# thomaspingel/neilpy

Hardware: AMD Instinct MI355X
Metric: Mcells/s through SMRF progressive_filter, 16384x16384 fp32 DEM (higher is better)
Workload: dtype f32

## Files before the change

### neilpy_amd/csrc/morph_incero.h

```cpp
#pragma once
#include "morph_ring.h"

namespace smrf {

#include "ero_inc.inc"
constexpr bool dil_cross_radii_are_rim_free() {
  for (int r = SMRF_INCERO_MIN_RADIUS; r <= SMRF_INCERO_MAX_RADIUS; ++r)
    if (smrf_dil_cross_has(4, r) != (kEroInc[r].n == 0)) return false;
  return true;
}
static_assert(dil_cross_radii_are_rim_free(), "smrf_dil_cross_has (pf_route.h) against ero_inc.inc");

enum { kIncEroPlain = 0, kIncEroMirrorSplit = 1, kIncEroMirrorCopy = 2 };
inline constexpr unsigned char kIncEroPlanKind[65] = {
    1, 1, 1, 1, 1, 1, 1, 1, 1, 1, 1, 1, 1, 1, 1, 1, 1,
    1, 1, 1, 1, 1, 1, 1, 1, 1, 1, 1, 1, 1, 1, 1, 1, 1,
    1, 1, 1, 1, 1, 1, 1, 1, 1, 1, 2, 2, 1, 1, 1, 1, 1,
    1, 1, 1, 1, 1, 1, 1, 1, 1, 1, 1, 1, 1, 1};
inline constexpr unsigned char kIncEroCrossLate[65] = {
    0, 0, 0, 0, 0, 0, 0, 0, 0, 0, 0, 0, 0, 0, 0, 0, 0,
    0, 0, 0, 0, 0, 0, 0, 0, 0, 0, 0, 0, 0, 0, 0, 0, 0,
    0, 0, 0, 0, 0, 1, 0, 0, 0, 0, 1, 1, 0, 0, 0, 1, 1,
    0, 0, 0, 0, 0, 0, 0, 0, 0, 0, 0, 0, 0, 0};
#ifndef SMRF_INCERO_MIRROR_GROUP
#define SMRF_INCERO_MIRROR_GROUP 2
#endif
constexpr int inc_ero_plan_kind(int radius) {
#ifdef SMRF_INCERO_PLAN
  return SMRF_INCERO_PLAN;
#else
  return kIncEroPlanKind[radius];
#endif
}
constexpr bool inc_ero_cross_late(int radius) {
#ifdef SMRF_INCERO_LATE
  return SMRF_INCERO_LATE;
#else
  return kIncEroCrossLate[radius] != 0;
#endif
}

template <typename T>
struct IncEroArgs {
  const T* e_prev;
  const T* last;
  T* out;
  int rows, cols;
  long long ld;
  int seg;
  int nt;
  int plain_tiles;
};

template <int R>
struct IncEroCfg {
  static constexpr int N = kEroInc[R].n;
  static constexpr int DY = kEroInc[R].reach;
  static constexpr int TW = 256, NP = 4, ROWS = 2 * NP;
  static constexpr int W = TW + 2 * DY;
  static constexpr int NPOS = (W + TW - 1) / TW;
  static constexpr int NACC = 2 * DY + ROWS;
  static constexpr int KIND = N > 0 ? inc_ero_plan_kind(R) : kIncEroPlain;
  static constexpr int NM = N / 2;
  static constexpr int G = KIND == kIncEroPlain ? 4 : SMRF_INCERO_MIRROR_GROUP;
  static constexpr int NJ = NP * N;
  static constexpr int dy(int k) { return kEroInc[R].p[k].dy; }
  static constexpr int dx(int k) { return kEroInc[R].p[k].dx; }
  static constexpr int slot(int j) { return 2 * (j / N) - dy(j % N) + DY; }
  static constexpr int mirror(int j) { return (j / N) * N + N - 1 - j % N; }
  static constexpr bool mirrored() {
    for (int k = 0; k < N; ++k)
      if (dy(k) != -dy(N - 1 - k) || dx(k) != dx(N - 1 - k) || dy(k) == 0) return false;
    return N % 2 == 0;
  }
  static constexpr short NONE = 32767;
  struct Item { short j; bool both; };
  struct Plan { short n, splits, copies; Item item[NJ > 0 ? NJ : 1]; short first[NACC]; };
  static constexpr Plan make_plan() {
    Plan pl{};
    for (int s = 0; s < NACC; ++s) pl.first[s] = NONE;
    auto emit = [&](int j, bool both) {
      for (int h = 0; h < (both ? 2 : 1); ++h)
        for (int b = 0; b < 2; ++b) {
          short& f = pl.first[slot(h ? mirror(j) : j) + b];
          if (f == NONE) f = pl.n;
        }
      pl.item[pl.n++] = Item{(short)j, both};
    };
    if constexpr (KIND == kIncEroPlain) {
      for (int s = 0; s < NACC; ++s)
        for (int j = 0; j < NJ; ++j)
          if (slot(j) == s) emit(j, false);
    } else {
      constexpr int NGR = NP * NM;
      auto jlo = [](int g) { return (g / NM) * N + NM + g % NM; };
      auto lo = [&](int g) { return slot(jlo(g)); };
      auto hi = [&](int g) { return slot(mirror(jlo(g))); };
      bool touched[NACC] = {}, done[NACC] = {};
      unsigned char state[NGR > 0 ? NGR : 1] = {};
      for (int g = 0; g < NGR; ++g) touched[lo(g)] = touched[lo(g) + 1] = touched[hi(g)] = touched[hi(g) + 1] = true;
      auto unready = [&](int g, int part) {
        int u = 0;
        for (int h = 0; h < 2; ++h)
          if (part >> h & 1)
            for (int b = 0; b < 2; ++b) {
// ... 16 lines not shown
          if (!part || unready(g, part)) continue;
          const int key = part & 1 ? lo(g) : hi(g);
          if (bg < 0 || key < bkey) bg = g, bpart = part, bkey = key;
        }
        if (bg < 0 && KIND == kIncEroMirrorSplit) {
          int bcnt = -1;
          for (int g = 0; g < NGR; ++g)
            for (int part = 1; part <= 2 && !state[g]; ++part) {
              if (unready(g, part)) continue;
              const int s = part == 1 ? lo(g) : hi(g);
              const bool was[2] = {done[s], done[s + 1]};
              done[s] = done[s + 1] = true;
              state[g] |= (unsigned char)part;
              int cnt = 0;
              for (int h = 0; h < NGR; ++h) {
                const int rest = 3 & ~state[h];
                const int a = lo(h) - s - ROWS, c = hi(h) - s - ROWS;
                if (rest && ((a >= -1 && a <= 1) || (c >= -1 && c <= 1)) && !unready(h, rest)) ++cnt;
              }
              state[g] = 0;
              done[s] = was[0], done[s + 1] = was[1];
              if (cnt > bcnt || (cnt == bcnt && s < bkey)) bg = g, bpart = part, bkey = s, bcnt = cnt;
            }
          ++pl.splits;
        } else if (bg < 0) {
          int bu = 0;
          for (int g = 0; g < NGR; ++g) {
            if (state[g]) continue;
            const int u = unready(g, 3);
            if (bg < 0 || u < bu || (u == bu && lo(g) < bkey)) bg = g, bpart = 3, bkey = lo(g), bu = u;
          }
        }
        run(bg, bpart);
        left -= bpart == 3 ? 2 : 1;
      }
    }
    return pl;
  }
  static constexpr Plan plan = make_plan();
  static constexpr int NI = plan.n;
  static constexpr int NG = (NI + G - 1) / G;
  static constexpr int gsize(int g) { const int n = NI - g * G; return n < 0 ? 0 : n > G ? G : n; }
  static constexpr bool plan_ok() {
    if (N > 0 && !mirrored()) return false;
    int seen[NJ > 0 ? NJ : 1] = {};
    for (int i = 0; i < NI; ++i) {
      ++seen[plan.item[i].j];
      if (plan.item[i].both) ++seen[mirror(plan.item[i].j)];
    }
    for (int j = 0; j < NJ; ++j)
      if (seen[j] != 1) return false;
    if (KIND == kIncEroPlain ? NI != NJ || plan.splits || plan.copies : NI != NP * NM + plan.splits) return false;
    if ((KIND == kIncEroMirrorSplit && plan.copies) || (KIND == kIncEroMirrorCopy && plan.splits)) return false;
    int late = 0;
    for (int s = 0; s < NACC; ++s) {
      int earliest = NONE, touches = 0;
      for (int i = NI - 1; i >= 0; --i)
        for (int h = 0; h < (plan.item[i].both ? 2 : 1); ++h)
          for (int b = 0; b < 2; ++b)
            if (slot(h ? mirror(plan.item[i].j) : plan.item[i].j) + b == s) { ++touches; earliest = i; }
      if (plan.first[s] != earliest) return false;
      if (touches && s + ROWS < NACC && plan.first[s + ROWS] != NONE && plan.first[s] >= plan.first[s + ROWS]) ++late;
    }
    return late == plan.copies;
  }
  static constexpr bool LATE = N > 0 && inc_ero_cross_late(R);
  static constexpr int DELTA = (ROWS - (2 * DY) % ROWS) % ROWS;
  static constexpr int LDS_CELLS = N > 0 ? 2 * NP * W : 1;
};

template <typename T, int R>
__global__ __launch_bounds__(256) void inc_erode_kernel(const IncEroArgs<T> a) {
  using C = IncEroCfg<R>;
  using T2 = typename Vec2<T>::type;
  constexpr int N = C::N, DY = C::DY, TW = C::TW, NP = C::NP, ROWS = C::ROWS, W = C::W, NPOS = C::NPOS, NACC = C::NACC, G = C::G;
  __shared__ T2 L[C::LDS_CELLS];
  const int tid = threadIdx.x;
  int bx, by;
  smrf_xcd_tile(a.plain_tiles, [] { return true; }, bx, by);
  const int x0 = bx * TW, x = x0 + tid;
  const int ys = by * a.seg, ye = min(a.rows, ys + a.seg);
  if (ys >= ye) return;
  const int xc = x < a.cols ? x : a.cols - 1;
  const int xl = smrf_fold(xc - 1, a.cols), xr = smrf_fold(xc + 1, a.cols);
  int cpos[NPOS];
  bool act[NPOS];
#pragma unroll
  for (int i = 0; i < NPOS; ++i) {
    act[i] = tid + i * TW < W;
    cpos[i] = smrf_fold(x0 - DY + tid + (act[i] ? i * TW : 0), a.cols);
  }
  T acc[NACC];
#pragma unroll
  for (int i = 0; i < NACC; ++i) acc[i] = ident<T>(false);

  static_assert(C::plan_ok(), "the batch plan");
  int o0 = ys - 2 * DY - C::DELTA;
  const int nb = (ye - o0 + ROWS - 1) / ROWS;
  RowFold rf(o0 + DY, a.rows);
  T2 pf[NP][NPOS];
  auto prefetch = [&]() {
#pragma unroll
    for (int p = 0; p < NP; ++p) {
      const T* ra = a.last + (long long)rf.at(2 * p) * a.ld;
      const T* rb = a.last + (long long)rf.at(2 * p + 1) * a.ld;
#pragma unroll
      for (int i = 0; i < NPOS; ++i)
        { pf[p][i].x = ra[cpos[i]]; pf[p][i].y = rb[cpos[i]]; }
    }
    rf.advance(ROWS);
  };
  if constexpr (N > 0) prefetch();

  T outv[ROWS];
  auto store_rows = [&](int ob) {
#pragma unroll
    for (int j = 0; j < ROWS; ++j)
      if (ob + j < ye && x < a.cols) smrf_store_out(a.out + (long long)(ob + j) * a.ld + x, outv[j], a.nt);
  };
  for (int b = 0; b < nb; ++b, o0 += ROWS) {
    const unsigned lds_b = (unsigned)(size_t)(__attribute__((address_space(3))) void*)(L + (b & 1) * NP * W + tid);
    if constexpr (N > 0) {
#pragma unroll
      for (int p = 0; p < NP; ++p)
#pragma unroll
        for (int i = 0; i < NPOS; ++i)
          lds_write2(lds_b + (unsigned)((p * W + (i < NPOS - 1 || act[i] ? i * TW : 0)) * (int)sizeof(T2)), pf[p][i]);
      lds_wait<0>();
      __syncthreads();
    }
    if (o0 - ROWS >= ys) store_rows(o0 - ROWS);
    const bool store = o0 >= ys;
    T ec[ROWS + 2], el[ROWS], er[ROWS];
    auto cross_loads = [&]() {
      RowFold rfe(o0 - 1, a.rows);
#pragma unroll
      for (int j = 0; j < ROWS + 2; ++j) {
        const T* row = a.e_prev + (long long)rfe.at(j) * a.ld;
        ec[j] = row[xc];
        if (j >= 1 && j <= ROWS) { el[j - 1] = row[xl]; er[j - 1] = row[xr]; }
      }
    };
    if constexpr (!C::LATE)
      if (store) cross_loads();
    if constexpr (N > 0) {
      __builtin_amdgcn_sched_barrier(0);
      prefetch();
      __builtin_amdgcn_sched_barrier(0);
      T old[NACC];
#pragma unroll
      for (int s = 0; s < NACC; ++s) old[s] = acc[s];
      [&]<int... S>(std::integer_sequence<int, S...>) {
        (([&] {
           if constexpr (C::plan.first[S] == C::NONE) acc[S] = S + ROWS < NACC ? old[S + ROWS] : ident<T>(false);
         }()),
         ...);
      }(std::make_integer_sequence<int, NACC>{});
      T2 rd[2 * G][2];
      auto issue = [&]<int I>(std::integral_constant<int, I>) {
        constexpr int J = C::plan.item[I].j, p = J / N, k = J % N;
        constexpr int offl = (p * W + DY - C::dx(k)) * (int)sizeof(T2), offr = (p * W + DY + C::dx(k)) * (int)sizeof(T2);
        rd[I % (2 * G)][0] = lds_read2<offl>(lds_b, T());
        rd[I % (2 * G)][1] = lds_read2<offr>(lds_b, T());
      };
      auto update = [&]<int S, int I>(std::integral_constant<int, S>, std::integral_constant<int, I>, const T& l, const T& r) {
        static_assert(S >= 0 && S < NACC, "slot outside the ring");
        if constexpr (C::plan.first[S] != I) op3_acc<false>(acc[S], l, r);
        else if constexpr (S + ROWS < NACC) acc[S] = op3<false>(old[S + ROWS], l, r);
        else acc[S] = op2<false>(l, r);
      };
      auto apply = [&]<int I>(std::integral_constant<int, I> i) {
        constexpr int s = C::slot(C::plan.item[I].j), m = C::slot(C::mirror(C::plan.item[I].j));
        update(std::integral_constant<int, s>{}, i, rd[I % (2 * G)][0].x, rd[I % (2 * G)][1].x);
        if constexpr (C::plan.item[I].both) update(std::integral_constant<int, m>{}, i, rd[I % (2 * G)][0].x, rd[I % (2 * G)][1].x);
        update(std::integral_constant<int, s + 1>{}, i, rd[I % (2 * G)][0].y, rd[I % (2 * G)][1].y);
        if constexpr (C::plan.item[I].both) update(std::integral_constant<int, m + 1>{}, i, rd[I % (2 * G)][0].y, rd[I % (2 * G)][1].y);
      };
      auto issue_group = [&]<int Gi>(std::integral_constant<int, Gi>) {
        [&]<int... I>(std::integer_sequence<int, I...>) {
          (issue(std::integral_constant<int, Gi * G + I>{}), ...);
        }(std::make_integer_sequence<int, C::gsize(Gi)>{});
      };
      auto apply_group = [&]<int Gi>(std::integral_constant<int, Gi>) {
        [&]<int... I>(std::integer_sequence<int, I...>) {
          (apply(std::integral_constant<int, Gi * G + I>{}), ...);
        }(std::make_integer_sequence<int, C::gsize(Gi)>{});
      };
      issue_group(std::integral_constant<int, 0>{});
      [&]<int... Gi>(std::integer_sequence<int, Gi...>) {
        (([&] {
           if constexpr (Gi + 1 < C::NG) {
             issue_group(std::integral_constant<int, Gi + 1>{});
             lds_wait<2 * C::gsize(Gi + 1)>();
           } else {
             lds_wait<0>();
           }
           apply_group(std::integral_constant<int, Gi>{});
         }()),
         ...);
      }(std::make_integer_sequence<int, C::NG>{});
    }
    if (store) {
      if constexpr (C::LATE) cross_loads();
#pragma unroll
      for (int j = 0; j < ROWS; ++j) {
        T m = op3<false>(ec[j + 1], el[j], er[j]);
        m = op3<false>(m, ec[j], ec[j + 2]);
        if constexpr (N > 0) m = op2<false>(m, acc[j]);
        outv[j] = m;
      }
    }
  }
  if (o0 - ROWS >= ys) store_rows(o0 - ROWS);
}

template <typename T, int R>
int inc_erode_launch(const IncEroArgs<T>& a_in, hipStream_t stream) {
  using C = IncEroCfg<R>;
  constexpr auto kern = inc_erode_kernel<T, R>;
  int resident;
  bool first;
  if (int rc = smrf_resident<kern>(C::TW, 0, resident, first)) return rc;
  if (first && smrf_sw().ring_debug)
    fprintf(stderr, "smrf inc erode: R=%d pairs=%d reach=%d LDS=%zu, %d workgroups/CU resident\n", R, C::N, C::DY,
            C::LDS_CELLS * 2 * sizeof(T), resident);
  IncEroArgs<T> a = a_in;
  const int strips = (a.cols + C::TW - 1) / C::TW;
  a.seg = smrf_seg_len(a.rows, strips, resident, smrf_sw().ring_rounds, 2 * C::DY + C::DELTA, C::ROWS, std::max(32, 4 * C::DY),
                       smrf_sw().seg_rule, a.seg);
  a.plain_tiles = smrf_sw().xcd_remap ? 0 : 1;
  dim3 grid(strips, (a.rows + a.seg - 1) / a.seg);
  hipLaunchKernelGGL(kern, grid, dim3(C::TW), 0, stream, a);
  SMRF_LAUNCH_CHECK();
  return SMRF_OK;
}

}
```

### neilpy_amd/csrc/morph_ring.h

```cpp
#pragma once
#include <algorithm>
#include <utility>

#include "smrf_common.h"

#ifndef SMRF_RING_G
#define SMRF_RING_G(ringregs) ((ringregs) > 132 ? 3 : (ringregs) > 100 ? 2 : 4)
#define SMRF_RING_G_OF(T, R, ringregs) (ring_tuned_g<T>(R) > 0 ? ring_tuned_g<T>(R) : SMRF_RING_G(ringregs))
#else
#define SMRF_RING_G_OF(T, R, ringregs) SMRF_RING_G(ringregs)
#endif
#ifndef SMRF_RING_TOP3
#define SMRF_RING_TOP3(T, R) ring_tuned_top3<T>(R)
#endif
#ifndef SMRF_RING_NP_MAX
#define SMRF_RING_NP_MAX 2
#endif
#ifndef SMRF_RING_XCD_REMAP
#define SMRF_RING_XCD_REMAP 1
#endif
#ifndef SMRF_RING_SLOPE_DEFAULT
#define SMRF_RING_SLOPE_DEFAULT 60
#endif
#ifndef SMRF_RING_OCC_DROP
// ... 313 lines not shown
  static constexpr int OCC_REG = INPLACE && SMRF_RING_INPLACE_OCC(T, R) > 0 ? SMRF_RING_INPLACE_OCC(T, R)
                                                                          : ring_occ_drop(OCC_EST, SMRF_RING_OCC_DROP_OF(T, R));
  static constexpr int WAVES = TW / 64;
  static constexpr int WG_LDS = (int)(160 * 1024 / LDS_BYTES) < 1 ? 1 : (int)(160 * 1024 / LDS_BYTES);
  static constexpr int OCC_LDS = WG_LDS * WAVES / 4 < 1 ? 1 : WG_LDS * WAVES / 4;
  static constexpr int OCC = OCC_REG < OCC_LDS ? OCC_REG : OCC_LDS;
  static constexpr int kA(int s) { int d = R - s - 2; return S::kidx(d < 0 ? -d : d); }
  static constexpr int kB(int s) { int d = R - s - 1; return S::kidx(d < 0 ? -d : d); }
  static constexpr int slot_group(int s) {
    if (s > R - 2) return NG;
    const int k = kA(s);
    return k == 0 ? 0 : (k - 1) / G;
  }
};

template <typename T, int R, int TW>
constexpr int ring_np() {
  using C1 = RingCfg<T, R, TW, 1>;
  constexpr int mx = C1::INPLACE && SMRF_RING_INPLACE_NP(T, R) > 0 ? SMRF_RING_INPLACE_NP(T, R)
                     : sizeof(T) == 4 ? SMRF_RING_NP_MAX_OF(T, R) : (ring_tuned_np_max<T>(R) / 2 < 1 ? 1 : ring_tuned_np_max<T>(R) / 2);
  constexpr int want = C1::OCC_REG * 4 / C1::WAVES < 1 ? 1 : C1::OCC_REG * 4 / C1::WAVES;
  if constexpr (mx >= 4) if (RingCfg<T, R, TW, 4>::WG_LDS >= want) return 4;
  if constexpr (mx >= 3) if (RingCfg<T, R, TW, 3>::WG_LDS >= want) return 3;
  if constexpr (mx >= 2) if (RingCfg<T, R, TW, 2>::WG_LDS >= want) return 2;
  return 1;
}
#define SMRF_RING_NP(T, R) ring_np<T, R, kRingTW>()


#ifndef SMRF_RING_BUF
#define SMRF_RING_BUF(T, R) ring_tuned_buf<T>(R)
#endif
#ifndef SMRF_RING_INPLACE_NOBUF
#define SMRF_RING_INPLACE_NOBUF(T, R) ((R) > 45)
#endif
template <typename T, int R, int TW, int NP>
constexpr bool ring_buf_on() { return SMRF_RING_BUF(T, R) && !(RingCfg<T, R, TW, NP>::INPLACE && SMRF_RING_INPLACE_NOBUF(T, R)); }
template <bool ON>
__device__ __forceinline__ int smrf_rare(int v) {
  if constexpr (ON) asm volatile("" : "+v"(v));
  return v;
}
using smrf_rsrc_t = __amdgpu_buffer_rsrc_t;
__device__ __forceinline__ smrf_rsrc_t smrf_make_rsrc(const void* p) {
  return __builtin_amdgcn_make_buffer_rsrc(const_cast<void*>(p), 0, -1, 0x00020000);
}
__device__ __forceinline__ float smrf_buf_load(smrf_rsrc_t r, unsigned voff, unsigned soff, float) {
  return __builtin_bit_cast(float, __builtin_amdgcn_raw_buffer_load_b32(r, (int)voff, (int)soff, 0));
}
__device__ __forceinline__ double smrf_buf_load(smrf_rsrc_t r, unsigned voff, unsigned soff, double) {
  return __builtin_bit_cast(double, __builtin_amdgcn_raw_buffer_load_b64(r, (int)voff, (int)soff, 0));
}
template <bool NT>
__device__ __forceinline__ void smrf_buf_store(smrf_rsrc_t r, unsigned voff, unsigned soff, float v) {
  __builtin_amdgcn_raw_buffer_store_b32(__builtin_bit_cast(unsigned, v), r, (int)voff, (int)soff, NT ? 2 : 0);
}
template <bool NT>
__device__ __forceinline__ void smrf_buf_store(smrf_rsrc_t r, unsigned voff, unsigned soff, double v) {
  typedef unsigned u2 __attribute__((ext_vector_type(2)));
  __builtin_amdgcn_raw_buffer_store_b64(__builtin_bit_cast(u2, v), r, (int)voff, (int)soff, NT ? 2 : 0);
}
__device__ __forceinline__ void smrf_buf_store_u8(smrf_rsrc_t r, unsigned voff, unsigned soff, uint8_t v) {
  __builtin_amdgcn_raw_buffer_store_b8(v, r, (int)voff, (int)soff, 0);
}

template <typename T>
__device__ __forceinline__ void smrf_store_out(T* p, T v, int nt) {
  if (nt) __builtin_nontemporal_store(v, p);
  else *p = v;
}
template <typename T>
__device__ __forceinline__ void smrf_flag_cell(const DiskArgs<T>& a, long long off, T lastval, T val) {
  const T diff = lastval - val;
  bool hit;
  if constexpr (sizeof(T) == 4) hit = diff > a.thr_lo;
  else hit = (double)diff > a.thr;
  if (a.dense) {
    a.mask[off] = hit ? 1 : 0;
    if (a.when != nullptr) a.when[off] = hit ? (uint8_t)a.widx : (uint8_t)0;
  } else if (hit) {
    a.mask[off] = 1;
    if (a.when != nullptr) a.when[off] = (uint8_t)a.widx;
  }
}

struct RowFold {
  int n, p;
  __device__ __forceinline__ RowFold(int y, int n_) : n(n_) {
    p = y % (2 * n);
    if (p < 0) p += 2 * n;
  }
  __device__ __forceinline__ int at(int i) const {
    int q = p + i;
    while (q >= 2 * n) q -= 2 * n;
    return q < n ? q : 2 * n - 1 - q;
  }
  __device__ __forceinline__ void advance(int d) {
    p += d;
    while (p >= 2 * n) p -= 2 * n;
  }
};

template <typename T, int R, bool DIL, int TW, int NP, int NPB, int OFF>
__device__ __forceinline__ void ring_base(typename Vec2<T>::type* const L, const int par, const int tid, const bool has_last,
                                          typename Vec2<T>::type (&v)[NP][RingCfg<T, R, TW, NP>::NPOS]) {
  using C = RingCfg<T, R, TW, NP>;
  using T2 = typename Vec2<T>::type;
  constexpr int WP = C::WP, NLEV = C::NLEV;
  constexpr int JB = C::JB, SB = C::slot_of(JB);
  constexpr int NA = (1 << JB) - 1;
  const unsigned lds_l = (unsigned)(size_t)(__attribute__((address_space(3))) void*)(L + tid + OFF);
  constexpr int PB = C::BASE_PB < NP ? C::BASE_PB : NP;
#pragma unroll
  for (int i = 0; i < NPB; ++i) {
    if (i < NPB - 1 || has_last) {
     const int pos = tid + OFF + i * TW;
#pragma unroll
     for (int p0 = 0; p0 < NP; p0 += PB) {
      T2 na[NP][NA];
#pragma unroll
      for (int p = p0; p < p0 + PB && p < NP; ++p) {
        const unsigned ad = lds_l + ((p * NLEV + par) * WP + i * TW) * (unsigned)sizeof(T2);
        [&]<int... Kk>(std::integer_sequence<int, Kk...>) {
          ((na[p][Kk] = lds_read2<(Kk + 1) * (int)sizeof(T2)>(ad, T())), ...);
        }(std::make_integer_sequence<int, NA>{});
      }
      lds_wait<0>();
#pragma unroll
      for (int p = p0; p < p0 + PB && p < NP; ++p) {
        const T2* n = na[p];
        T2 m = v[p][i];
        if constexpr (C::INC) {
          m.x = op2<DIL>(m.x, n[0].x); m.y = op2<DIL>(m.y, n[0].y);
          if constexpr (JB >= 2) {
            if constexpr (C::stored(1)) { constexpr int s1 = C::slot_of(1); L[(p * NLEV + s1) * WP + pos] = m; }
            m.x = op3<DIL>(m.x, n[1].x, n[2].x); m.y = op3<DIL>(m.y, n[1].y, n[2].y);
          }
          if constexpr (JB == 3) {
            if constexpr (C::stored(2)) { constexpr int s2 = C::slot_of(2); L[(p * NLEV + s2) * WP + pos] = m; }
            m.x = op3<DIL>(m.x, n[3].x, n[4].x); m.y = op3<DIL>(m.y, n[3].y, n[4].y);
            m.x = op3<DIL>(m.x, n[5].x, n[6].x); m.y = op3<DIL>(m.y, n[5].y, n[6].y);
          }
        } else {
        if constexpr (JB == 1) { m.x = op2<DIL>(m.x, n[0].x); m.y = op2<DIL>(m.y, n[0].y); }
        if constexpr (JB >= 2) {
          m.x = op3<DIL>(m.x, n[0].x, n[1].x); m.y = op3<DIL>(m.y, n[0].y, n[1].y);
          m.x = op2<DIL>(m.x, n[2].x); m.y = op2<DIL>(m.y, n[2].y);
        }
        if constexpr (JB == 3) {
          m.x = op3<DIL>(m.x, n[3].x, n[4].x); m.y = op3<DIL>(m.y, n[3].y, n[4].y);
          m.x = op3<DIL>(m.x, n[5].x, n[6].x); m.y = op3<DIL>(m.y, n[5].y, n[6].y);
        }
        }
        v[p][i] = m;
        L[(p * NLEV + SB) * WP + pos] = m;
      }
      __builtin_amdgcn_sched_barrier(0);
     }
    }
  }
}

template <typename T, int R, bool DIL, int TW, int NP, int NPB, int OFF>
__device__ __forceinline__ void ring_upper(typename Vec2<T>::type* const L, const int tid, const bool has_last,
                                           typename Vec2<T>::type (&v)[NP][RingCfg<T, R, TW, NP>::NPOS]) {
  using C = RingCfg<T, R, TW, NP>;
// ... 382 lines not shown
           constexpr int ka = C::kA(Sl), kb = C::kB(Sl);
           if constexpr ((ka - 1) / G == GI) {
             constexpr int src = Sl + 2 <= R - 2 ? Sl + 2 : R - 1 + ((Sl + 2 - (R - 1)) + 2 * P) % M;
             acc[Sl] = op3<DIL>(acc[src], ra[ka], rb[kb]);
           }
         }()), ...);
      }(std::make_integer_sequence<int, R - 1>{});
      [&]<int... Jr>(std::integer_sequence<int, Jr...>) {
        (([&] {
           constexpr int j = R - 2 - Jr;
           constexpr int ka = S::kidx(j + 1), kb = S::kidx(j);
           if constexpr ((kb - 1) / G == GI) {
             constexpr int reg = R - 1 + (j + 2 + 2 * P) % M;
             op3_acc<DIL>(acc[reg], ra[ka], rb[kb]);
           }
         }()), ...);
      }(std::make_integer_sequence<int, R - 1>{});
    };
    [&]<int... GI>(std::integer_sequence<int, GI...>) {
      (([&] { if constexpr (GI < NG) lk.template issue<GI>(); }()), ...);
    }(std::make_integer_sequence<int, D - 1>{});
    ra[0] = own[P].x;
    rb[0] = own[P].y;
    outv[2 * P] = op2<DIL>(acc[0], ra[0]);
    constexpr bool SD = C::SLOT_DELAY && NG >= 2;
    [&]<int... GI>(std::integer_sequence<int, GI...>) {
      (([&] {
         if constexpr (GI + D - 1 < NG) lk.template issue<GI + D - 1>();
         lds_wait<C::inflight_after(GI), (C::FUSE_MODE != 0)>();
         lk.template reduce<GI>();
         constexpr int GS = SD ? GI - 1 : GI;
         if constexpr (GS == (KR1 - 1) / G) outv[2 * P + 1] = op3<DIL>(acc[1], ra[KR1], rb[0]);
         if constexpr (!SD && GI == NG - 1) __builtin_amdgcn_s_setprio(0);
         if constexpr (GS >= 0) slots(std::integral_constant<int, GS>{});
       }()), ...);
    }(std::make_integer_sequence<int, NG>{});
    if constexpr (SD) {
      __builtin_amdgcn_s_setprio(0);
      if constexpr (NG - 1 == (KR1 - 1) / G) outv[2 * P + 1] = op3<DIL>(acc[1], ra[KR1], rb[0]);
      slots(std::integral_constant<int, NG - 1>{});
    }
    acc[R - 1 + (2 * P) % M] = op2<DIL>(ra[0], rb[KR1]);
    acc[R - 1 + (1 + 2 * P) % M] = rb[0];
    __builtin_amdgcn_sched_barrier(0);
  };
  [&]<int... P>(std::integer_sequence<int, P...>) {
    (pair_body(std::integral_constant<int, P>{}), ...);
  }(std::make_integer_sequence<int, NP>{});
  {
    constexpr int ROT = (2 * NP) % M;
    if constexpr (ROT != 0) {
      SMRF_MARK("turn");
      T t[M];
#pragma unroll
      for (int i = 0; i < M; ++i) t[i] = acc[R - 1 + (i + ROT) % M];
      if constexpr (sizeof(T) == 4 && SMRF_RING_TURN_ASM(T, R)) {
#pragma unroll
        for (int i = 0; i < M; ++i) asm volatile("v_mov_b32 %0, %1" : "=v"(acc[R - 1 + i]) : "v"(t[i]));
      } else {
#pragma unroll
        for (int i = 0; i < M; ++i) acc[R - 1 + i] = t[i];
      }
    }
  }
}

template <typename T, int R, bool DIL, int TW, int NP, int NPB, int OFF, typename Sync>
__device__ __forceinline__ void ring_build_consume(typename Vec2<T>::type* const L, const int par, const int tid,
                                                   const bool has_last,
                                                   typename Vec2<T>::type (&v)[NP][RingCfg<T, R, TW, NP>::NPOS],
                                                   T (&acc)[2 * R], T (&outv)[2 * NP], Sync&& phase_sync) {
  __builtin_amdgcn_s_setprio(kRingBuildPrio);
  ring_base<T, R, DIL, TW, NP, NPB, OFF>(L, par, tid, has_last, v);
  phase_sync();
  if constexpr (RingCfg<T, R, TW, NP>::J > RingCfg<T, R, TW, NP>::JB) {
    ring_upper<T, R, DIL, TW, NP, NPB, OFF>(L, tid, has_last, v);
    phase_sync();
  }
  __builtin_amdgcn_s_setprio(0);
  ring_consume<T, R, DIL, TW, NP>(L, par, tid, acc, outv);
}

#ifndef SMRF_CROSS_NP
#define SMRF_CROSS_NP(R) ((R) == 16 ? 2 : 0)
#endif
#ifndef SMRF_CROSS_OCC
#define SMRF_CROSS_OCC(R) ((R) == 36 ? 2 : 3)
#endif
template <int R, int TW, int NP>
constexpr int ring_cross_occ() {
  using C = RingCfg<float, R, TW, NP>;
  constexpr int o = SMRF_CROSS_OCC(R) > 0 ? SMRF_CROSS_OCC(R) : C::OCC_REG;
  return o < C::OCC_LDS ? o : C::OCC_LDS;
}

template <typename T, int R, bool DIL, int TW, int NP>
__global__ __launch_bounds__(TW, (RingCfg<T, R, TW, NP>::OCC))
void ring_kernel(const DiskArgs<T> a) {
  constexpr bool CROSS = false;
#include "ring_kernel_body.inc"
}

template <int R, int TW, int NP>
__global__ __launch_bounds__(TW, (ring_cross_occ<R, TW, NP>()))
void ring_cross_kernel(const DiskArgs<float> a) {
  using T = float;
  constexpr bool DIL = true, CROSS = true;
#include "ring_kernel_body.inc"
}

template <typename T, int R, bool DIL, int NP, bool CROSS = false>
int ring_launch_np(const DiskArgs<T>& a_in, hipStream_t stream, bool probe_only, int* seg_if_launched) {
  constexpr int TW = kRingTW;
  using C = RingCfg<T, R, TW, NP>;
  constexpr auto kern = [] {
    if constexpr (CROSS) return ring_cross_kernel<R, TW, NP>;
    else return ring_kernel<T, R, DIL, TW, NP>;
  }();
  constexpr int occ = [] {
    if constexpr (CROSS) return ring_cross_occ<R, TW, NP>();
    else return (int)C::OCC;
  }();
  int resident;
  bool first;
  if (int rc = smrf_resident<kern>(TW, C::LDS_BYTES, resident, first)) return rc;
  if (first && smrf_sw().ring_debug)
    fprintf(stderr, "smrf ring: R=%d %s%s NP=%d G=%d%s LDS=%zu built for %d waves/SIMD, %d workgroups/CU resident\n", R,
            sizeof(T) == 4 ? "f32" : "f64", CROSS ? " dilate of the cross" : DIL ? " dilate" : " erode", NP, C::G, C::INPLACE ? " in-place" : "", C::LDS_BYTES,
            occ, resident);
  DiskArgs<T> a = a_in;
  const int strips = (a.cols + TW - 1) / TW;
  const int slope_env = smrf_sw().ring_slope;
  const int slope = slope_env >= 0 ? slope_env : (sizeof(T) == 4 && 256 % strips == 0 ? SMRF_RING_SLOPE_DEFAULT : 0);
  int max_rows = 0;
  if constexpr (ring_buf_on<T, R, TW, NP>()) {
    const long long rowb = (long long)a.ld * (long long)sizeof(T);
    const long long most = ((1ll << 31) - 1) / rowb - (4 * R + 4 * C::ROWS);
    if (most < C::ROWS) return smrf_fail(SMRF_E_UNSUPPORTED, "raster rows of %lld bytes are too long for this build", rowb);
    max_rows = (int)most;
  }
  const SmrfRingPlan p = smrf_ring_plan(a.out_rows, strips, R, C::ROWS, resident, smrf_sw().ring_rounds, smrf_sw().seg_rule,
                                        slope, a_in.seg, max_rows);
  a.seg = p.seg;
  a.seg_cls = p.seg_cls;
  std::copy(p.seg_first, p.seg_first + 8, a.seg_first);
  std::copy(p.seg_row0, p.seg_row0 + 8, a.seg_row0);
  std::copy(p.seg_len, p.seg_len + 8, a.seg_len);
  a.plain_tiles = smrf_sw().xcd_remap ? 0 : 1;
  if (seg_if_launched) *seg_if_launched = p.seg_cls ? p.seg_equal : p.seg;
  if (probe_only) return SMRF_OK;
  dim3 grid(strips, p.grid_y);
  hipLaunchKernelGGL(kern, grid, dim3(TW), C::LDS_BYTES, stream, a);
  SMRF_LAUNCH_CHECK();
  return SMRF_OK;
}

template <typename T, int R, bool DIL>
int ring_launch(const DiskArgs<T>& a_in, hipStream_t stream) {
  constexpr int TW = kRingTW;
  constexpr int NP = SMRF_RING_NP(T, R);
  if constexpr (ring_tuned_inplace_dual<T>(R) && SMRF_RING_INPLACE(T, R)) {
    constexpr int NPI = SMRF_RING_INPLACE_NP(T, R);
    static_assert(NPI != NP, "a dual radius needs two different instances");
    static_assert(RingCfg<T, R, TW, NPI>::INPLACE && !RingCfg<T, R, TW, NP>::INPLACE, "dual instances mixed up");
    const int mode = smrf_sw().ring_dual;
    int seg = a_in.seg;
    if (mode != 0 && a_in.seg <= 0) {
// ... 16 lines not shown
```

### neilpy_amd/csrc/ring_kernel_body.inc

```
  static_assert(!CROSS || (DIL && sizeof(T) == 4), "cross on load: the fp32 dilation only");
  using C = RingCfg<T, R, TW, NP>;
  using T2 = typename Vec2<T>::type;
  constexpr int WP = C::WP, ROWS = C::ROWS, NLEV = C::NLEV;
  static_assert(sizeof(T) == 4 || NP <= 2, "fp64 ring instances are validated for at most two row pairs per batch");
  extern __shared__ __attribute__((aligned(16))) unsigned char smrf_lds[];
  T2* const L = reinterpret_cast<T2*>(smrf_lds);

  const int tid = threadIdx.x;
  int bx, by;
  smrf_xcd_tile(!SMRF_RING_XCD_REMAP || a.plain_tiles, [&] { return a.seg_cls == 0; }, bx, by);
#ifdef SMRF_RING_DBG_CLOCK
  const unsigned long long dbg_t0 = __builtin_amdgcn_s_memtime(), dbg_q0 = __builtin_amdgcn_s_memrealtime();
#endif
#ifdef SMRF_RING_DBG_TS
  const unsigned long long dbg_ts0 = __builtin_amdgcn_s_memrealtime();
#endif
  const int x0 = bx * TW;
  const int x = x0 + tid;
  int ys, ye;
  if (a.seg_cls > 0) {
    int cls = 0;
    for (int c = 1; c < a.seg_cls; ++c) cls += by >= a.seg_first[c] ? 1 : 0;
    ys = a.out_row0 + a.seg_row0[cls] + (by - a.seg_first[cls]) * a.seg_len[cls];
    ye = min(a.out_row0 + a.out_rows, ys + a.seg_len[cls]);
    if (ys >= ye) return;
  } else {
    ys = a.out_row0 + by * a.seg;
    ye = min(a.out_row0 + a.out_rows, ys + a.seg);
  }
  constexpr int NPOS = C::NPOS, W = C::W;
  const bool has_last = tid + (NPOS - 1) * TW < W;
  int cpos[NPOS];
#pragma unroll
  for (int i = 0; i < NPOS; ++i) cpos[i] = smrf_fold(x0 - R + tid + (tid + i * TW < W ? i * TW : 0), a.cols);
  const int last_in = a.in_rows - 1;
  using H = HaloCfg<T, R, TW, NP>;
  constexpr bool BAL = H::OK;
  HaloLane hl;
  hl.wave = __builtin_amdgcn_readfirstlane(tid >> 6);
  {
    const int h = (hl.wave % H::NH) * 64 + (tid & 63);
    hl.act = BAL && h < H::HW;
    hl.pos = hl.act ? TW + h : TW;
  }
  const int hcol = smrf_fold(x0 - R + hl.pos, a.cols);
  int cposl[NPOS], cposr[NPOS], hcoll = 0, hcolr = 0;
  if constexpr (CROSS) {
#pragma unroll
    for (int i = 0; i < NPOS; ++i) { cposl[i] = smrf_fold(cpos[i] - 1, a.cols); cposr[i] = smrf_fold(cpos[i] + 1, a.cols); }
    hcoll = smrf_fold(hcol - 1, a.cols);
    hcolr = smrf_fold(hcol + 1, a.cols);
  }
  static_assert(TW == kRingTW, "the table is shared by the workgroup's four waves: workgroup barriers between the phases");
  auto phase_sync = [&]() { __syncthreads(); };
  const bool flag = a.mask != nullptr;
  const int xc = x < a.cols ? x : a.cols - 1;

  T acc[2 * R];
#pragma unroll
  for (int i = 0; i < 2 * R; ++i) acc[i] = ident<T>(DIL);

  T2 pf[NP][NPOS];
  T2 pfh[H::NJ];
  constexpr int NPX = CROSS ? (BAL ? 1 : NPOS) : 1, NJX = CROSS ? H::NJ : 1;
  T pxc[NPX][ROWS + 2], pxl[NPX][ROWS], pxr[NPX][ROWS];
  T phc[NJX][4], phl[NJX][2], phr[NJX][2];
  T outv[ROWS], lastv[ROWS];
#pragma unroll
  for (int i = 0; i < ROWS; ++i) { outv[i] = T(0); lastv[i] = T(0); }

  constexpr int DELTA = (ROWS - (2 * R) % ROWS) % ROWS;
  const int ystart = ys - R - DELTA;
  constexpr int UP = CROSS ? 1 : 0;
  RowFold rf(ystart - UP, a.img_rows);
  constexpr bool BUF = ring_buf_on<T, R, TW, NP>();
  constexpr bool RARE = C::INPLACE && SMRF_RING_RARE_OPAQUE(T, R);
  const int bi = max(0, ystart - UP - a.in_row0);
  const int bl = max(0, ys - 2 * R - DELTA - a.out_row0);
  const int bo = ys - a.out_row0;
  const unsigned rowb = (unsigned)a.ld * (unsigned)sizeof(T);
  const smrf_rsrc_t rs_in = smrf_make_rsrc(a.in + (long long)bi * a.ld);
  const smrf_rsrc_t rs_out = smrf_make_rsrc(a.out + (long long)bo * a.ld);
  const smrf_rsrc_t rs_last = smrf_make_rsrc(flag ? a.last + (long long)bl * a.ld : nullptr);
  const smrf_rsrc_t rs_mask = smrf_make_rsrc(flag ? a.mask + (long long)bo * a.ld : nullptr);
  const smrf_rsrc_t rs_when = smrf_make_rsrc(flag && a.when != nullptr ? a.when + (long long)bo * a.ld : nullptr);
  unsigned cposb[NPOS], hcolb = 0, xb = 0, xcb = 0;
  if constexpr (BUF) {
#pragma unroll
    for (int i = 0; i < NPOS; ++i) cposb[i] = (unsigned)cpos[i] * (unsigned)sizeof(T);
    hcolb = (unsigned)hcol * (unsigned)sizeof(T);
    xb = (unsigned)x * (unsigned)sizeof(T);
    xcb = (unsigned)xc * (unsigned)sizeof(T);
  }
  auto cross_fill = [&](auto&& cell) __attribute__((always_inline)) {
#pragma unroll
    for (int i = 0; i < NPX; ++i) {
      const unsigned cb = (unsigned)cpos[i] * (unsigned)sizeof(T), lb = (unsigned)cposl[i] * (unsigned)sizeof(T), rb = (unsigned)cposr[i] * (unsigned)sizeof(T);
#pragma unroll
      for (int k = 0; k < ROWS + 2; ++k) pxc[i][k] = cell(k, cpos[i], cb);
#pragma unroll
      for (int k = 0; k < ROWS; ++k) { pxl[i][k] = cell(k + 1, cposl[i], lb); pxr[i][k] = cell(k + 1, cposr[i], rb); }
    }
    if constexpr (BAL) {
      const unsigned cb = (unsigned)hcol * (unsigned)sizeof(T), lb = (unsigned)hcoll * (unsigned)sizeof(T), rb = (unsigned)hcolr * (unsigned)sizeof(T);
#pragma unroll
      for (int j = 0; j < NJX; ++j) {
        const int q = hl.wave + H::WAVES * j;
        const int pq = q < H::NQ ? q / H::NH : 0;
#pragma unroll
        for (int k = 0; k < 4; ++k) phc[j][k] = cell(2 * pq + k, hcol, cb);
#pragma unroll
        for (int k = 0; k < 2; ++k) { phl[j][k] = cell(2 * pq + 1 + k, hcoll, lb); phr[j][k] = cell(2 * pq + 1 + k, hcolr, rb); }
      }
    }
  };
  auto cross_reduce = [&]() __attribute__((always_inline)) {
    if constexpr (CROSS) {
#pragma unroll
      for (int p = 0; p < NP; ++p) {
#pragma unroll
        for (int i = 0; i < NPX; ++i) {
          pf[p][i].x = op3<false>(op3<false>(pxc[i][2 * p + 1], pxl[i][2 * p], pxr[i][2 * p]), pxc[i][2 * p], pxc[i][2 * p + 2]);
          pf[p][i].y = op3<false>(op3<false>(pxc[i][2 * p + 2], pxl[i][2 * p + 1], pxr[i][2 * p + 1]), pxc[i][2 * p + 1], pxc[i][2 * p + 3]);
        }
      }
      if constexpr (BAL) {
#pragma unroll
        for (int j = 0; j < NJX; ++j) {
          pfh[j].x = op3<false>(op3<false>(phc[j][1], phl[j][0], phr[j][0]), phc[j][0], phc[j][2]);
          pfh[j].y = op3<false>(op3<false>(phc[j][2], phl[j][1], phr[j][1]), phc[j][1], phc[j][3]);
        }
      }
    }
  };
  auto prefetch = [&]() {
    const int l0 = rf.p - a.in_row0;
    if constexpr (CROSS) {
      if (rf.p + ROWS + 2 <= rf.n && l0 >= 0 && l0 + ROWS + 1 <= last_in) {
        SMRF_MARK("prefetch");
        if constexpr (BUF) {
          const unsigned s0 = (unsigned)(l0 - bi) * rowb;
          cross_fill([&](int k, int, unsigned cb) { return smrf_buf_load(rs_in, cb, s0 + (unsigned)k * rowb, T()); });
        } else {
          const T* r0 = a.in + (long long)l0 * a.ld;
          cross_fill([&](int k, int c, unsigned) { return r0[(long long)k * a.ld + c]; });
        }
      } else {
        SMRF_MARK("rare");
        cross_fill([&](int k, int c, unsigned) {
          int l = rf.at(k) - a.in_row0;
          l = l < 0 ? 0 : (l > last_in ? last_in : l);
          return a.in[(long long)l * a.ld + smrf_rare<RARE>(c)];
        });
      }
      SMRF_MARK("prefetch");
      rf.advance(ROWS);
      return;
    }
    if (rf.p + ROWS <= rf.n && l0 >= 0 && l0 + ROWS - 1 <= last_in) {
      SMRF_MARK("prefetch");
      if constexpr (BUF) {
        const unsigned s0 = (unsigned)(l0 - bi) * rowb;
#pragma unroll
        for (int p = 0; p < NP; ++p) {
#pragma unroll
          for (int i = 0; i < (BAL ? 1 : NPOS); ++i) {
            pf[p][i].x = smrf_buf_load(rs_in, cposb[i], s0 + (unsigned)(2 * p) * rowb, T());
            pf[p][i].y = smrf_buf_load(rs_in, cposb[i], s0 + (unsigned)(2 * p + 1) * rowb, T());
          }
        }
        if constexpr (BAL) {
#pragma unroll
          for (int j = 0; j < H::NJ; ++j) {
            const int q = hl.wave + H::WAVES * j;
            const int pq = q < H::NQ ? q / H::NH : 0;
            pfh[j].x = smrf_buf_load(rs_in, hcolb, s0 + (unsigned)(2 * pq) * rowb, T());
            pfh[j].y = smrf_buf_load(rs_in, hcolb, s0 + (unsigned)(2 * pq + 1) * rowb, T());
          }
        }
      } else {
      const T* r0 = a.in + (long long)l0 * a.ld;
#pragma unroll
      for (int p = 0; p < NP; ++p) {
#pragma unroll
        for (int i = 0; i < (BAL ? 1 : NPOS); ++i) {
          pf[p][i].x = r0[(long long)(2 * p) * a.ld + cpos[i]];
          pf[p][i].y = r0[(long long)(2 * p + 1) * a.ld + cpos[i]];
        }
      }
      if constexpr (BAL) {
#pragma unroll
        for (int j = 0; j < H::NJ; ++j) {
          const int q = hl.wave + H::WAVES * j;
          const int pq = q < H::NQ ? q / H::NH : 0;
          pfh[j].x = r0[(long long)(2 * pq) * a.ld + hcol];
          pfh[j].y = r0[(long long)(2 * pq + 1) * a.ld + hcol];
        }
      }
      }
    } else {
      SMRF_MARK("rare");
#pragma unroll
      for (int p = 0; p < NP; ++p) {
        int la = rf.at(2 * p) - a.in_row0;
        int lb = rf.at(2 * p + 1) - a.in_row0;
        la = la < 0 ? 0 : (la > last_in ? last_in : la);
// ... 201 lines not shown
```

Baseline: 4409.

## Replace left/right cross-stencil loads with wave DPP shifts plus one edge load

The plus-shaped cross stencil used to load the left and right neighbour columns from global memory for every row. It now loads only the centre column plus one per-wave edge value and builds the neighbours with DPP wave shifts (row_shr/row_shl with bound control), which removes two gathered loads per row. The late cross-load schedule table and the cross NP setting for R=16 are retuned to match. The risk is correctness: the 0x138/0x130 DPP codes must give full-wave shifts whose lane 0 and lane 63 pick up the edge value, and partial tiles and the changed cpos activity condition must still map to the right columns.

Result: no change. 4410 (median of 2 runs) (+0.0%).

```diff
diff --git a/neilpy_amd/csrc/morph_incero.h b/neilpy_amd/csrc/morph_incero.h
--- a/neilpy_amd/csrc/morph_incero.h
+++ b/neilpy_amd/csrc/morph_incero.h
@@ -20,7 +20,7 @@
 inline constexpr unsigned char kIncEroCrossLate[65] = {
     0, 0, 0, 0, 0, 0, 0, 0, 0, 0, 0, 0, 0, 0, 0, 0, 0,
     0, 0, 0, 0, 0, 0, 0, 0, 0, 0, 0, 0, 0, 0, 0, 0, 0,
-    0, 0, 0, 0, 0, 1, 0, 0, 0, 0, 1, 1, 0, 0, 0, 1, 1,
+    0, 0, 0, 0, 0, 0, 0, 0, 0, 0, 1, 1, 0, 1, 1, 1, 1,
     0, 0, 0, 0, 0, 0, 0, 0, 0, 0, 0, 0, 0, 0};
 #ifndef SMRF_INCERO_MIRROR_GROUP
 #define SMRF_INCERO_MIRROR_GROUP 2
@@ -203,7 +203,8 @@
   const int ys = by * a.seg, ye = min(a.rows, ys + a.seg);
   if (ys >= ye) return;
   const int xc = x < a.cols ? x : a.cols - 1;
-  const int xl = smrf_fold(xc - 1, a.cols), xr = smrf_fold(xc + 1, a.cols);
+  const int xw = x0 + (tid & ~63);
+  const int xe = (tid & 32) == 0 ? smrf_fold(min(xw, a.cols - 1) - 1, a.cols) : smrf_fold(min(xw + 63, a.cols - 1) + 1, a.cols);
   int cpos[NPOS];
   bool act[NPOS];
 #pragma unroll
@@ -252,14 +253,14 @@
     }
     if (o0 - ROWS >= ys) store_rows(o0 - ROWS);
     const bool store = o0 >= ys;
-    T ec[ROWS + 2], el[ROWS], er[ROWS];
+    T ec[ROWS + 2], ee[ROWS];
     auto cross_loads = [&]() {
       RowFold rfe(o0 - 1, a.rows);
 #pragma unroll
       for (int j = 0; j < ROWS + 2; ++j) {
         const T* row = a.e_prev + (long long)rfe.at(j) * a.ld;
         ec[j] = row[xc];
-        if (j >= 1 && j <= ROWS) { el[j - 1] = row[xl]; er[j - 1] = row[xr]; }
+        if (j >= 1 && j <= ROWS) ee[j - 1] = row[xe];
       }
     };
     if constexpr (!C::LATE)
@@ -325,7 +326,7 @@
       if constexpr (C::LATE) cross_loads();
 #pragma unroll
       for (int j = 0; j < ROWS; ++j) {
-        T m = op3<false>(ec[j + 1], el[j], er[j]);
+        T m = op3<false>(ec[j + 1], wave_lower(ec[j + 1], ee[j]), wave_upper(ec[j + 1], ee[j]));
         m = op3<false>(m, ec[j], ec[j + 2]);
         if constexpr (N > 0) m = op2<false>(m, acc[j]);
         outv[j] = m;
diff --git a/neilpy_amd/csrc/morph_ring.h b/neilpy_amd/csrc/morph_ring.h
--- a/neilpy_amd/csrc/morph_ring.h
+++ b/neilpy_amd/csrc/morph_ring.h
@@ -419,6 +419,13 @@
     a.mask[off] = 1;
     if (a.when != nullptr) a.when[off] = (uint8_t)a.widx;
   }
+}
+
+__device__ __forceinline__ float wave_lower(float v, float edge) {
+  return __builtin_bit_cast(float, __builtin_amdgcn_update_dpp(__builtin_bit_cast(int, edge), __builtin_bit_cast(int, v), 0x138, 0xf, 0xf, false));
+}
+__device__ __forceinline__ float wave_upper(float v, float edge) {
+  return __builtin_bit_cast(float, __builtin_amdgcn_update_dpp(__builtin_bit_cast(int, edge), __builtin_bit_cast(int, v), 0x130, 0xf, 0xf, false));
 }
 
 struct RowFold {
@@ -967,7 +974,7 @@
 }
 
 #ifndef SMRF_CROSS_NP
-#define SMRF_CROSS_NP(R) ((R) == 16 ? 2 : 0)
+#define SMRF_CROSS_NP(R) 0
 #endif
 #ifndef SMRF_CROSS_OCC
 #define SMRF_CROSS_OCC(R) ((R) == 36 ? 2 : 3)
diff --git a/neilpy_amd/csrc/ring_kernel_body.inc b/neilpy_amd/csrc/ring_kernel_body.inc
--- a/neilpy_amd/csrc/ring_kernel_body.inc
+++ b/neilpy_amd/csrc/ring_kernel_body.inc
@@ -32,7 +32,7 @@
   const bool has_last = tid + (NPOS - 1) * TW < W;
   int cpos[NPOS];
 #pragma unroll
-  for (int i = 0; i < NPOS; ++i) cpos[i] = smrf_fold(x0 - R + tid + (tid + i * TW < W ? i * TW : 0), a.cols);
+  for (int i = 0; i < NPOS; ++i) cpos[i] = smrf_fold(x0 - R + tid + (tid + i * TW < W + (CROSS ? 1 : 0) ? i * TW : 0), a.cols);
   const int last_in = a.in_rows - 1;
   using H = HaloCfg<T, R, TW, NP>;
   constexpr bool BAL = H::OK;
@@ -44,10 +44,12 @@
     hl.pos = hl.act ? TW + h : TW;
   }
   const int hcol = smrf_fold(x0 - R + hl.pos, a.cols);
-  int cposl[NPOS], cposr[NPOS], hcoll = 0, hcolr = 0;
+  int cpose[NPOS], hcoll = 0, hcolr = 0;
   if constexpr (CROSS) {
-#pragma unroll
-    for (int i = 0; i < NPOS; ++i) { cposl[i] = smrf_fold(cpos[i] - 1, a.cols); cposr[i] = smrf_fold(cpos[i] + 1, a.cols); }
+    const int w0 = tid & ~63;
+#pragma unroll
+    for (int i = 0; i < NPOS; ++i)
+      cpose[i] = smrf_fold(x0 - R + w0 + (w0 + i * TW < W ? i * TW : 0) + ((tid & 32) == 0 ? -1 : 64), a.cols);
     hcoll = smrf_fold(hcol - 1, a.cols);
     hcolr = smrf_fold(hcol + 1, a.cols);
   }
@@ -63,7 +65,7 @@
   T2 pf[NP][NPOS];
   T2 pfh[H::NJ];
   constexpr int NPX = CROSS ? (BAL ? 1 : NPOS) : 1, NJX = CROSS ? H::NJ : 1;
-  T pxc[NPX][ROWS + 2], pxl[NPX][ROWS], pxr[NPX][ROWS];
+  T pxc[NPX][ROWS + 2], pxe[NPX][ROWS];
   T phc[NJX][4], phl[NJX][2], phr[NJX][2];
   T outv[ROWS], lastv[ROWS];
 #pragma unroll
@@ -95,11 +97,11 @@
   auto cross_fill = [&](auto&& cell) __attribute__((always_inline)) {
 #pragma unroll
     for (int i = 0; i < NPX; ++i) {
-      const unsigned cb = (unsigned)cpos[i] * (unsigned)sizeof(T), lb = (unsigned)cposl[i] * (unsigned)sizeof(T), rb = (unsigned)cposr[i] * (unsigned)sizeof(T);
+      const unsigned cb = (unsigned)cpos[i] * (unsigned)sizeof(T), eb = (unsigned)cpose[i] * (unsigned)sizeof(T);
 #pragma unroll
       for (int k = 0; k < ROWS + 2; ++k) pxc[i][k] = cell(k, cpos[i], cb);
 #pragma unroll
-      for (int k = 0; k < ROWS; ++k) { pxl[i][k] = cell(k + 1, cposl[i], lb); pxr[i][k] = cell(k + 1, cposr[i], rb); }
+      for (int k = 0; k < ROWS; ++k) pxe[i][k] = cell(k + 1, cpose[i], eb);
     }
     if constexpr (BAL) {
       const unsigned cb = (unsigned)hcol * (unsigned)sizeof(T), lb = (unsigned)hcoll * (unsigned)sizeof(T), rb = (unsigned)hcolr * (unsigned)sizeof(T);
@@ -120,8 +122,9 @@
       for (int p = 0; p < NP; ++p) {
 #pragma unroll
         for (int i = 0; i < NPX; ++i) {
-          pf[p][i].x = op3<false>(op3<false>(pxc[i][2 * p + 1], pxl[i][2 * p], pxr[i][2 * p]), pxc[i][2 * p], pxc[i][2 * p + 2]);
-          pf[p][i].y = op3<false>(op3<false>(pxc[i][2 * p + 2], pxl[i][2 * p + 1], pxr[i][2 * p + 1]), pxc[i][2 * p + 1], pxc[i][2 * p + 3]);
+          const T ca = pxc[i][2 * p + 1], cb = pxc[i][2 * p + 2];
+          pf[p][i].x = op3<false>(op3<false>(ca, wave_lower(ca, pxe[i][2 * p]), wave_upper(ca, pxe[i][2 * p])), pxc[i][2 * p], cb);
+          pf[p][i].y = op3<false>(op3<false>(cb, wave_lower(cb, pxe[i][2 * p + 1]), wave_upper(cb, pxe[i][2 * p + 1])), ca, pxc[i][2 * p + 3]);
         }
       }
       if constexpr (BAL) {
```
